# User-tian/Conan

Measured on AMD Instinct MI355X. Metric: chunks/sec (80 ms chunk, 16 kHz), all streams summed; p50 per-chunk latency beside it, higher is better.
Workload: dtype f32 (3×bf16-limb products, f32 accumulate)

## Files before the change

conan_amd/csrc/api.hip:

```cpp
#include "streams.h"

static thread_local std::string g_err;

template <typename F>
static int guarded(F&& f) {
  try {
    f();
    const hipError_t le = hipGetLastError();
    if (le != hipSuccess) throw ch::Error(CONAN_ERR_HIP, std::string("HIP launch error: ") + hipGetErrorString(le));
    return CONAN_OK;
  } catch (const ch::Error& e) {
    g_err = e.what();
    return e.code;
  } catch (const std::exception& e) {
    g_err = e.what();
    return CONAN_ERR_INVALID;
  }
}

static void validate_cfg(const conan_cfg& c) {
  if (c.abi_version != CONAN_HIP_ABI_VERSION) throw Error(CONAN_ERR_INVALID, "conan_cfg.abi_version mismatch");
  if (c.models & CONAN_MODEL_HIFIGAN) {
    if (c.voc_num_ups < 1 || c.voc_num_ups > CONAN_MAX_UPS) throw Error(CONAN_ERR_INVALID, "voc_num_ups");
    if (c.voc_num_resblocks < 1 || c.voc_num_resblocks > 3) throw Error(CONAN_ERR_UNSUPPORTED, "1..3 resblock branches supported");
// ... 187 lines not shown
}

int conan_streams_create_opts(conan_ctx* ctx, int max_slots, int max_frames, int max_ref_frames, const conan_streams_opts* opts,
                              conan_streams** out) {
  return guarded([&] {
    if (!ctx || !out) throw Error(CONAN_ERR_INVALID, "null argument");
    int arith = CONAN_ARITH_AUTO, flags = 0;
    if (opts) {
      if (opts->abi_version != CONAN_HIP_ABI_VERSION) throw Error(CONAN_ERR_INVALID, "conan_streams_opts.abi_version mismatch");
      for (int r : opts->reserved) if (r != 0) throw Error(CONAN_ERR_INVALID, "conan_streams_opts.reserved must be 0");
      arith = opts->arith; flags = opts->flags;
      if (opts->reserved0 != 0) throw Error(CONAN_ERR_INVALID, "conan_streams_opts.reserved0 must be 0");
      if (flags & ~(CONAN_STREAMS_FUSED_DECODER_BLOCKS | CONAN_STREAMS_SEPARATE_SMALL_STEPS | CONAN_STREAMS_FIXED_PLAN | CONAN_STREAMS_SHARED_DEVICE)) throw Error(CONAN_ERR_INVALID, "conan_streams_opts.flags: unknown bits");
      if (arith != CONAN_ARITH_AUTO && arith != CONAN_ARITH_F32 && arith != CONAN_ARITH_LIMB) throw Error(CONAN_ERR_INVALID, "conan_streams_opts.arith: 0 (auto), 1 (f32) or 2 (limb)");
    }
    if (!ctx->finalized) throw Error(CONAN_ERR_STATE, "conan_ctx_finalize must run before conan_streams_create");
    if (max_slots < 1 || max_frames < 1) throw Error(CONAN_ERR_INVALID, "max_slots / max_frames");
    HIP_CHECK(hipSetDevice(ctx->device));
    conan_streams* s = new conan_streams();
    try {
      s->parse_dev_plan(opts ? opts->dev_plan : nullptr);
      s->fixed_plan = (flags & CONAN_STREAMS_FIXED_PLAN) != 0; s->shared_device = (flags & CONAN_STREAMS_SHARED_DEVICE) != 0;
      s->ctx = ctx; s->live = &device_live_streams(ctx->device); s->live->fetch_add(1); s->max_slots = max_slots; s->max_frames = std::max(max_frames, ctx->cfg.emf_segment); s->max_ref = std::max(4, max_ref_frames);
      s->d_slots = (int*)s->alloc(max_slots + cnk::kSlotTablePad); s->d_ident = (int*)s->alloc(max_slots + 1); s->d_zero = (int*)s->alloc(max_slots);
      s->d_lens = (int*)s->alloc(max_slots); s->d_lens2 = (int*)s->alloc(max_slots);
      s->d_codes = (int*)s->alloc((size_t)max_slots * s->max_frames * 2);
      s->sk_slab_floats = 8ll << 20; s->sk_max_tiles = 4096;
      for (int w = 0; w < 3; ++w) { s->sk_slab[w] = s->alloc((size_t)s->sk_slab_floats); s->sk_counters[w] = (int*)s->alloc(s->sk_max_tiles); }
      for (int w = 0; w < 2; ++w) s->rb_sched[w] = (int*)s->alloc(4);
      for (int w = 0; w < 3; ++w) s->cp_ticket[w] = (int*)s->alloc(4);
      { const char* e = s->dev("RESERVE_CUS"); s->reserve_cus = e ? atoi(e) : 0; }
      { const char* e = s->dev("ROWCONV"); s->use_rowconv = !(e && e[0] == '0'); }
      s->rb_merge = s->dev("RB_NOMERGE") == nullptr;
      if (arith == CONAN_ARITH_LIMB && !((ctx->cfg.models & CONAN_MODEL_HIFIGAN) && ctx->has_limb_weights))
        throw Error(CONAN_ERR_UNSUPPORTED, "arith = limb: this context holds no bf16-limb weights (no HiFi-GAN model, or a vocoder configuration without limb kernels)");
      s->arith_auto = arith == CONAN_ARITH_AUTO;
      s->rb_limb = arith == CONAN_ARITH_LIMB || (arith == CONAN_ARITH_AUTO && ctx->has_limb_weights && s->dev("RB_NOLIMB") == nullptr);
      s->opt_flags = flags;
      s->mega_single = !(s->opt_flags & CONAN_STREAMS_SEPARATE_SMALL_STEPS);
      { const char* e = s->dev("FENCED"); s->fenced = e && e[0] == '1'; }
      { const char* e = s->dev("DEC_MEGA"); s->use_mega = !(e && e[0] == '0'); }
      { const char* e = s->dev("MEGA_GRID"); if (e && atoi(e) > 0) s->mega_grid = std::min(atoi(e), ctx->num_cu); }
      { const char* e = s->dev("FRONT_CUSTRIDE"); if (e && atoi(e) >= 2) s->use_mega = false; }
      { const char* e = s->dev("MEGA_GS"); if (e && (atoi(e) == 4 || atoi(e) == 8 || atoi(e) == 16)) s->mega_gs = atoi(e); }
      { const char* e = s->dev("MEGA_NARROW"); if (e && e[0] == '0') s->mega_narrow_ksplit = false; }
      s->mega_bar = reinterpret_cast<unsigned*>(s->alloc(16 * (size_t)(ctx->num_cu + 2)));
      s->mega_x = reinterpret_cast<unsigned*>(s->alloc(256 + 32 * 64));

      {
        HIP_CHECK(hipHostMalloc((void**)&s->h_guard, 64, hipHostMallocMapped));
        memset(s->h_guard, 0, 64);
        unsigned* hdev = nullptr;
        HIP_CHECK(hipHostGetDevicePointer((void**)&hdev, s->h_guard, 0));
        s->d_guard = reinterpret_cast<unsigned*>(s->alloc(16));
        HIP_CHECK(hipMemcpy(s->d_guard + 2, &hdev, sizeof(hdev), hipMemcpyHostToDevice));
      }
      s->slot_seen.assign(max_slots, 0); s->has_ref.assign(max_slots, 0); s->voice_of.assign(max_slots, -1); s->voc_fresh.assign(max_slots, 1); s->wav_out.voc_samples.assign(max_slots, 0); s->wav_in.in_fmt.assign(max_slots, 0); s->wav_out.out_fmt.assign(max_slots, 0);
      s->pin.init((size_t)max_slots + cnk::kSlotTablePad);
      s->pos_emf = (int*)s->alloc(max_slots); s->pos_dec = (int*)s->alloc(max_slots); s->pos_voc = (int*)s->alloc(max_slots);
      std::vector<int> id(max_slots);
      for (int i = 0; i < max_slots; ++i) id[i] = i;
      HIP_CHECK(hipMemcpy(s->d_ident, id.data(), max_slots * sizeof(int), hipMemcpyHostToDevice));
      s->wav_in.fe_slot.assign(max_slots, conan_streams::FeSlot());
      if ((ctx->cfg.models & 7) == 7) {
        const int seg = ctx->cfg.emf_segment, rc = ctx->cfg.emf_right_context, hop = ctx->hop;
        s->wav_in.fe_LA = ch::next_pow2(2048 + seg * hop);
// ... 578 lines not shown
```

conan_amd/csrc/kernels.h:

```cpp
#pragma once
#include <hip/hip_runtime.h>
#include <stdint.h>
#include <stdlib.h>

#include "voice_layout.h"

namespace cnk {

inline const char* dev_getenv(const char* name) {
#ifdef CONAN_DEV_SWITCHES
  return getenv(name);
#else
  (void)name;
  return nullptr;
#endif
}
#define HIP_CHECK(x) ::ch::hip_check((x), #x)


struct TRef {
  float* base;
  long long slot_stride;
  int C;
  int lmask;
// ... 102 lines not shown
  const int* assign;
  int assign_per;
  int wr_max;
  float* slab; int* counters;
  long long slab_floats; int max_counters;
};
bool conv_limb_supported(const ConvArgs& a);
int conv_limb_shape(const ConvArgs* p, int nprob, int num_cu, int plan_n = 0, bool tail_split = false);
bool launch_conv_limb(const ConvLimbGroup& g, int shape, int num_cu, hipStream_t st);
int conv_limb_tail_slices(const ConvArgs& a, int shape, int num_cu);
const char* conv_limb_name(int shape);

struct RBProb {
  const float* w1; const float* w2;
  const float* b1; const float* b2;
  const unsigned short* w1l; const unsigned short* w2l;
  TRef x;
  TRef y;
  int k, dil;
};
struct RBArgs {
  RBProb p[3];
  const int* slots; const int* pos;
  const int* tiles;
  int ntiles;
  int* sched;
  int nprob, n, T;
  int tiles_per_slot;
  int order[3];
  float slope;
  int merge;
  TRef ymean;
  unsigned long long* dbg;
};
bool resblock_fused_supported(int C, int kmax, int span_max);
int resblock_fused_rows(int C, int T, int n, int ksum, int kmax, int num_cu);
bool launch_resblock_fused(const RBArgs& a, int C, int rows, int num_cu, hipStream_t st);
bool resblock_fused_can_merge(int C, int rows);
const char* resblock_fused_name(int C, int rows, bool merge = false);
const int* resblock_tiles(const RBArgs& a, int ro, int* total_out);
bool resblock_limb_supported(int C, int kmax, int span_max);
constexpr int kResblockLimbMaxSlots = 256;
int resblock_limb_rows(int C, int span_max);
bool launch_resblock_limb(const RBArgs& a, int C, int rows, int num_cu, hipStream_t st);
bool resblock_limb_can_merge(int C, int rows);
const char* resblock_limb_name(int C, int rows, bool merge = false);


struct RPProb {
  const float* w1; const float* w2;
  const float* b1; const float* b2;
  TRef x, y;
  TRef xh;
  int k, dil;
};
struct RPArgs {
  RPProb p[3];
  const int* slots; const int* pos;
  const int* tiles; int ntiles;
  int* sched;
  float* xb;
  unsigned* xflag; unsigned* mbox; unsigned* xcount;
  int nprob, n, T;
  float slope;
  unsigned* guard;
  int fault;
// ... 414 lines not shown
```

conan_amd/csrc/resblock_limb.hip:

```cpp
#include <algorithm>
#include <cstring>
#include <type_traits>

#include "kernels.h"

#define RL_MAX_SLOTS 256

#ifndef RL_HELPER_PRIO
#define RL_HELPER_PRIO 3
#endif
#ifndef RL_MATRIX_PRIO
#define RL_MATRIX_PRIO 0
#endif
#ifndef RL_STAMPS
#define RL_STAMPS 0
#endif

#ifdef RL_ABLATE_W
#define RL_WOFF(x) 0
#define RL_WOFF2(a_, b_) (b_)
#else
#define RL_WOFF(x) (x)
#define RL_WOFF2(a_, b_) (a_)
#endif
// ... 177 lines not shown
            __builtin_amdgcn_sched_group_barrier(0x100, 1, 0);
          }
        } else {
          __builtin_amdgcn_sched_group_barrier(0x008, NRW * NCW, 0);
        }
      }
      __builtin_amdgcn_sched_group_barrier(0x020, 3 * NCW, 0);
      __builtin_amdgcn_sched_barrier(0);
    }
  }
}

}

#define RL_SEL(br_, f) ((br_) == 0 ? a.p[0].f : ((br_) == 1 ? a.p[1].f : a.p[2].f))

template <int C, int NR2, int SPAN, bool MERGE>
__global__ __launch_bounds__(512, 2) void resblock_limb_kernel(const RBArgs a) {
  using G = RLGeom<C, NR2, SPAN>;
  constexpr int LDB = G::LDB;
  __shared__ __attribute__((aligned(16))) u16 lds[G::LDS_U16 + 16 + 4 * RL_MAX_SLOTS];
  u16* const win = lds;
  u16* const xt = lds + 3 * G::PLW;
  float* const accimg = reinterpret_cast<float*>(xt);
  int* const meta = reinterpret_cast<int*>(lds + G::LDS_U16);
  int* const sptab = meta + 8;
  const int tid = threadIdx.x;
  const int lane = tid & 63;
  const int wave = __builtin_amdgcn_readfirstlane(tid >> 6);
  const int ntiles = a.ntiles;
  const float slope = a.slope;
  const int T = a.T;
  constexpr bool merge = MERGE;
  const int np = a.nprob;

  if (wave >= 4) {
    const int ht = tid - 256;
    __builtin_amdgcn_s_setprio(RL_HELPER_PRIO);
    auto hbar = [&]() __attribute__((always_inline)) { asm volatile("s_waitcnt lgkmcnt(0)\n\ts_barrier" ::: "memory"); };
    constexpr int NIT = (G::WR_MAX * G::C4 + 255) / 256;
    float4 wv[NIT];
    int wtotal = 0, wzr = 0;
    auto win_issue = [&](const int p, const int i, const int t0, const int slot, const int pos) __attribute__((always_inline)) {
      const int k = RL_SEL(p, k), d = RL_SEL(p, dil);
      const int wr = G::XT_ROWS + (k - 1) * d;
      const int tw0 = t0 - (k - 1) - (k - 1) * d;
      const int xmode = a.p[0].x.mode, xrate = a.p[0].x.rate;
      const float* xb = RL_SEL(p, x.base) + (long long)(xmode == 0 ? slot : i) * RL_SEL(p, x.slot_stride);
      const unsigned rbase = (xmode == 0 ? (unsigned)pos * (unsigned)xrate : 0u) + (unsigned)(RL_SEL(p, x.off) + tw0);
      const unsigned rmask = xmode == 0 ? (unsigned)RL_SEL(p, x.lmask) : 0xffffffffu;
      wtotal = wr * G::C4;
#pragma unroll
      for (int u = 0; u < NIT; ++u) {
        const int idx = ht + 256 * u;
        const int w = idx / G::C4, c4 = idx - w * G::C4;
        const unsigned row = (rbase + (unsigned)w) & rmask;
        wv[u] = idx < wtotal ? rl_gload4(xb + (long long)row * C + c4 * 4) : make_float4(0.f, 0.f, 0.f, 0.f);
      }
      const long long abs0 = (xmode == 0 ? (long long)pos * xrate : 0ll) + t0 - (k - 1);
      wzr = abs0 >= 0 ? 0 : (abs0 < -(long long)G::XT_ROWS ? G::XT_ROWS : (int)-abs0);
    };
    auto win_write = [&]() __attribute__((always_inline)) {
#pragma unroll
      for (int u = 0; u < NIT; ++u) {
        const int idx = ht + 256 * u;
        const int w = idx / G::C4, c4 = idx - w * G::C4;
        unsigned h[2], m[2], l[2];
        rl_split2(rl_lrelu2((f32x2){wv[u].x, wv[u].y}, slope), h[0], m[0], l[0]);
        rl_split2(rl_lrelu2((f32x2){wv[u].z, wv[u].w}, slope), h[1], m[1], l[1]);
        if (idx < wtotal) {
          u16* dst = win + w * LDB + c4 * 4;
          *reinterpret_cast<uint2*>(dst) = make_uint2(h[0], h[1]);
          *reinterpret_cast<uint2*>(dst + G::PLW) = make_uint2(m[0], m[1]);
          *reinterpret_cast<uint2*>(dst + 2 * G::PLW) = make_uint2(l[0], l[1]);
        }
      }
      if (ht == 0) meta[0] = wzr;
    };
    constexpr int NOUT = (G::RO * G::C4) / 256;
// ... 43 lines not shown
          else {
            float4 sm = osum[MERGE ? u : 0];
            if (op == 0) sm = v; else { sm.x += v.x; sm.y += v.y; sm.z += v.z; sm.w += v.w; }
            osum[MERGE ? u : 0] = sm;
            if (op == np - 1) {
              const float dn = (float)np;
              if (np > 1) { sm.x /= dn; sm.y /= dn; sm.z /= dn; sm.w /= dn; }
              sm.x = sm.x > 0.f ? sm.x : sm.x * slope; sm.y = sm.y > 0.f ? sm.y : sm.y * slope;
              sm.z = sm.z > 0.f ? sm.z : sm.z * slope; sm.w = sm.w > 0.f ? sm.w : sm.w * slope;
              rl_gstore4(oyb + (long long)((oyr0 + (unsigned)r) & oym) * oyC + oc4 * 4, sm);
            }
          }
        }
      }
    };
#if RL_STAMPS
    const unsigned long long h_t0 = __builtin_amdgcn_s_memtime();
    unsigned long long h_t[6] = {0, 0, 0, 0, 0, 0};
#define RL_HT(i_) h_t[i_] = __builtin_amdgcn_s_memtime() - h_t0
#else
#define RL_HT(i_)
#endif
    int dv0 = 0;
    if (wave == 4 && lane == 0) dv0 = __hip_atomic_fetch_add(a.sched, 1, __ATOMIC_RELAXED, __HIP_MEMORY_SCOPE_AGENT);
    for (int e = ht; e < a.n; e += 256) {
      const int sl = a.slots ? *(gci)(a.slots + e) : e;
      sptab[2 * e] = sl; sptab[2 * e + 1] = a.pos ? *(gci)(a.pos + sl) : 0;
    }
    const int tps = a.tiles_per_slot, per_prob = a.n * tps;
    auto decode = [&](const int e, int& p, int& i, int& t0) __attribute__((always_inline)) {
      if constexpr (!MERGE) {
        const int b = e / per_prob, rem = e - b * per_prob;
        p = b == 0 ? a.order[0] : (b == 1 ? a.order[1] : a.order[2]);
        i = rem / tps; t0 = (rem - i * tps) * G::RO;
      } else {
        const int g = e / np;
        p = e - g * np; i = g / tps; t0 = (g - i * tps) * G::RO;
      }
    };
    int cur = -1, p = -1, i = 0, t0 = 0;
    if (wave == 4) {
      cur = __builtin_amdgcn_readfirstlane(dv0) * (merge ? np : 1);
      if (cur >= ntiles) cur = -1;
      if (cur >= 0) decode(cur, p, i, t0);
      if (lane == 0) { meta[1] = cur; meta[2] = p; meta[3] = 0; }
    }
    RL_HT(0);
    asm volatile("s_waitcnt lgkmcnt(0)\n\ts_barrier" ::: "memory");
    RL_HT(1);
    if (wave != 4) {
      cur = __builtin_amdgcn_readfirstlane(meta[1]);
      if (cur >= 0) decode(cur, p, i, t0);
    }
    if (cur >= 0) {
    int slot = __builtin_amdgcn_readfirstlane(sptab[2 * i]), pos = __builtin_amdgcn_readfirstlane(sptab[2 * i + 1]);
    win_issue(p, i, t0, slot, pos);
    RL_HT(2);
    int gen = 1;
    int dv = 0, dnext = -1;
    auto draw_issue = [&](const int have, const int idx_prev, const int p_prev) __attribute__((always_inline)) {
      if (wave == 4 && lane == 0 && have) {
        if (merge && p_prev != np - 1) dnext = idx_prev + 1;
        else { dnext = -1; dv = __hip_atomic_fetch_add(a.sched, 1, __ATOMIC_RELAXED, __HIP_MEMORY_SCOPE_AGENT); }
      }
    };
    auto draw_take = [&](const int have) __attribute__((always_inline)) {
      int idx = -1;
      if (!have) return idx;
      if (wave == 4) {
        const int drawn = dv * (merge ? np : 1);
        idx = __builtin_amdgcn_readfirstlane(dnext >= 0 ? dnext : drawn);
        if (idx >= ntiles) idx = -1;
        if (lane == 0) {
          meta[1] = idx;
          asm volatile("s_waitcnt lgkmcnt(0)" ::: "memory");
          __hip_atomic_store(&meta[3], gen, __ATOMIC_RELEASE, __HIP_MEMORY_SCOPE_WORKGROUP);
        }
      } else {
        while (__hip_atomic_load(&meta[3], __ATOMIC_ACQUIRE, __HIP_MEMORY_SCOPE_WORKGROUP) != gen) __builtin_amdgcn_s_sleep(4);
        idx = __builtin_amdgcn_readfirstlane(meta[1]);
      }
      ++gen;
      return idx;
    };
    const bool deep = ntiles >= 5 * (int)gridDim.x * (merge ? np : 1);
    auto stage = [&](const int e) __attribute__((always_inline)) {
      int pe, ie, te;
      decode(e, pe, ie, te);
      win_issue(pe, ie, te, __builtin_amdgcn_readfirstlane(sptab[2 * ie]), __builtin_amdgcn_readfirstlane(sptab[2 * ie + 1]));
      return pe;
    };
    int nxt = -1, pn = -1;
    if (deep) {
      draw_issue(1, cur, p);
      nxt = draw_take(1);
    }
    RL_HT(3);
    win_write();
    RL_HT(4);
    hbar();
    RL_HT(5);
#if RL_STAMPS
    if (a.dbg && blockIdx.x == 0 && wave == 4 && lane == 0) { unsigned long long* q = a.dbg + 256 * 4 + 12; for (int e = 0; e < 6; ++e) q[e] = h_t[e]; }
#endif
    bool pending = false;
    for (;;) {
      const bool have = deep ? nxt >= 0 : true;
      if (deep && nxt >= 0) pn = stage(nxt);
      draw_issue(have, deep ? nxt : cur, deep ? pn : p);
      if (pending) out_store();
      int nn = -1;
      if (!deep) {
        nxt = draw_take(have); pn = -1;
        if (nxt >= 0) pn = stage(nxt);
      }
      if (ht == 0) meta[2] = nxt >= 0 ? pn : -1;
      hbar();
      hbar();
      if (nxt >= 0) win_write();
      hbar();
      hbar();
      out_fetch(p, i, t0, slot, pos);
      pending = true;
      if (deep) nn = draw_take(have);
      if (nxt < 0) break;
      cur = nxt;
      decode(cur, p, i, t0);
      slot = __builtin_amdgcn_readfirstlane(sptab[2 * i]); pos = __builtin_amdgcn_readfirstlane(sptab[2 * i + 1]);
      nxt = nn;
    }
    if (pending) out_store();
    }
    if (ht == 0) {
      const int d = __hip_atomic_fetch_add(a.sched + 1, 1, __ATOMIC_RELAXED, __HIP_MEMORY_SCOPE_AGENT);
      if (d == (int)gridDim.x - 1) {
        __hip_atomic_store(a.sched, 0, __ATOMIC_RELAXED, __HIP_MEMORY_SCOPE_AGENT);
        __hip_atomic_store(a.sched + 1, 0, __ATOMIC_RELAXED, __HIP_MEMORY_SCOPE_AGENT);
      }
    }
    return;
  }

  if (RL_MATRIX_PRIO) __builtin_amdgcn_s_setprio(RL_MATRIX_PRIO);
  auto bar = [&]() __attribute__((always_inline)) { asm volatile("s_waitcnt lgkmcnt(0)\n\ts_barrier" ::: "memory"); };
  const int wc = wave % (4 / G::RSPLIT);
  const int wr = wave / (4 / G::RSPLIT);
  const int ct0 = wc * G::NCW;
  const int lr = lane & 15, lg = lane >> 4;
#if RL_STAMPS
  unsigned long long st_gemm = 0, st_t0 = __builtin_amdgcn_s_memtime(), st_r0 = __builtin_amdgcn_s_memrealtime(), st_bar = 0, st_b3 = 0, st_b1 = 0, st_b4 = 0, st_b2 = 0, st_e1 = 0, st_e2 = 0, st_tiles = 0, st_head = 0, st_pre = 0, st_mid = 0;
#define RL_T() __builtin_amdgcn_s_memtime()
#define RL_BAR(acc_) do { const unsigned long long q0_ = RL_T(); bar(); const unsigned long long q1_ = RL_T(); acc_ += q1_ - q0_; st_bar += q1_ - q0_; } while (0)
#define RL_GEMM(...) do { const unsigned long long s0_ = RL_T(); __VA_ARGS__; asm volatile("s_nop 0" ::"v"(acc[0][0][0])); st_gemm += RL_T() - s0_; } while (0)
#else
#define RL_BAR(acc_) bar()
#define RL_GEMM(...) __VA_ARGS__
#endif
  f32x4 bw[G::RING][G::NCW][3];
  bar();
  int p = __builtin_amdgcn_readfirstlane(meta[2]);
  if (p < 0) return;
  {
    const long long cs = (long long)(RL_SEL(p, k) + 1) * G::KB * G::BLK;
    rl_prefetch_w<G::NCW, G::RING>(bw, RL_SEL(p, w1l) + (long long)ct0 * cs + lane * 8, cs);
  }
  bar();
#if RL_STAMPS
  st_head = RL_T() - st_t0;
#endif
  while (p >= 0) {
#if RL_STAMPS
    const unsigned long long top_ = RL_T();
#endif
    const int k = RL_SEL(p, k), d = RL_SEL(p, dil);
    const u16* const w1 = RL_SEL(p, w1l);
    const u16* const w2 = RL_SEL(p, w2l);
    const float* const b1 = RL_SEL(p, b1);
    const long long ct_stride = (long long)(k + 1) * G::KB * G::BLK;
    const int zrows = __builtin_amdgcn_readfirstlane(meta[0]);
    f32x4 b1v[G::NCW];
#pragma unroll
    for (int c = 0; c < G::NCW; ++c) b1v[c] = rl_gload(b1 + (ct0 + c) * 16 + 4 * lg);
    int pn;
    {
      f32x4 acc[G::NRW1][G::NCW];
#pragma unroll
      for (int r = 0; r < G::NRW1; ++r)
#pragma unroll
        for (int c = 0; c < G::NCW; ++c) acc[r][c] = (f32x4){0.f, 0.f, 0.f, 0.f};
      const int rt0 = wr * G::NRW1;
#if RL_STAMPS
      st_pre += RL_T() - top_;
#endif
      RL_GEMM(rl_gemm<G::NRW1, G::NCW, LDB, G::KB, G::RING>(win, G::PLW, rt0 * 16, d, k, w1 + (long long)ct0 * ct_stride + lane * 8, ct_stride,
                                                           w2 + (long long)ct0 * ct_stride + lane * 8, ct_stride, acc, bw, lane));
      RL_BAR(st_b3);
#if RL_STAMPS
      const unsigned long long e1_0 = RL_T();
#endif
      auto epilogue1 = [&](auto zr_c) __attribute__((always_inline)) {
        constexpr bool ZR = decltype(zr_c)::value;
#pragma unroll
        for (int c = 0; c < G::NCW; ++c) {
          const int col = (ct0 + c) * 16 + 4 * lg;
#pragma unroll
          for (int r = 0; r < G::NRW1; ++r) {
            if (rt0 + r < G::NR1) {
              const int m = (rt0 + r) * 16 + lr;
              unsigned h[2], mm[2], l[2];
              const f32x4 v = acc[r][c] + b1v[c];
              rl_split2(rl_lrelu2((f32x2){v[0], v[1]}, slope), h[0], mm[0], l[0]);
              rl_split2(rl_lrelu2((f32x2){v[2], v[3]}, slope), h[1], mm[1], l[1]);
              const bool zr = ZR && m < zrows;
              u16* dst = xt + m * LDB + col;
              *reinterpret_cast<uint2*>(dst) = zr ? make_uint2(0u, 0u) : make_uint2(h[0], h[1]);
              *reinterpret_cast<uint2*>(dst + G::PLX) = zr ? make_uint2(0u, 0u) : make_uint2(mm[0], mm[1]);
              *reinterpret_cast<uint2*>(dst + 2 * G::PLX) = zr ? make_uint2(0u, 0u) : make_uint2(l[0], l[1]);
            }
          }
        }
      };
      if (zrows > 0) epilogue1(std::true_type{}); else epilogue1(std::false_type{});
#if RL_STAMPS
      asm volatile("s_waitcnt lgkmcnt(0)" ::: "memory"); st_e1 += RL_T() - e1_0; ++st_tiles;
#endif
    }
    RL_BAR(st_b1);
#if RL_STAMPS
    const unsigned long long mid_ = RL_T();
#endif
    pn = __builtin_amdgcn_readfirstlane(meta[2]);
    const int pnx = pn >= 0 ? pn : p;
    const long long csn = (long long)(RL_SEL(pnx, k) + 1) * G::KB * G::BLK;
    const u16* const w1n = RL_SEL(pnx, w1l) + (long long)ct0 * csn + lane * 8;
    {
      f32x4 acc[G::NRW2][G::NCW];
#pragma unroll
      for (int r = 0; r < G::NRW2; ++r)
#pragma unroll
        for (int c = 0; c < G::NCW; ++c) acc[r][c] = (f32x4){0.f, 0.f, 0.f, 0.f};
      const int rt0 = wr * G::NRW2;
#if RL_STAMPS
      st_mid += RL_T() - mid_;
#endif
      RL_GEMM(rl_gemm<G::NRW2, G::NCW, LDB, G::KB, G::RING>(xt, G::PLX, rt0 * 16, 1, k, w2 + (long long)ct0 * ct_stride + lane * 8, ct_stride,
                                                           w1n, csn, acc, bw, lane));
      RL_BAR(st_b4);
#if RL_STAMPS
      const unsigned long long e2_0 = RL_T();
#endif
#pragma unroll
      for (int c = 0; c < G::NCW; ++c) {
        const int col = (ct0 + c) * 16 + 4 * lg;
#pragma unroll
        for (int r = 0; r < G::NRW2; ++r) {
          if (rt0 + r < NR2) *reinterpret_cast<f32x4*>(accimg + ((rt0 + r) * 16 + lr) * G::LDA + col) = acc[r][c];
        }
      }
#if RL_STAMPS
      asm volatile("s_waitcnt lgkmcnt(0)" ::: "memory"); st_e2 += RL_T() - e2_0;
#endif
    }
    RL_BAR(st_b2);
    p = pn;
  }
#if RL_STAMPS
  if (a.dbg && tid == 0) {
    unsigned long long* o = a.dbg + blockIdx.x * 4;
    if (blockIdx.x == 0) { unsigned long long* q = a.dbg + 256 * 4; q[0] = st_b3; q[1] = st_b1; q[2] = st_b4; q[3] = st_b2; q[4] = st_e1; q[5] = st_e2; q[6] = st_tiles; q[7] = st_gemm; q[8] = __builtin_amdgcn_s_memtime() - st_t0; q[9] = st_head; q[10] = st_pre; q[11] = st_mid; }
    o[0] = st_gemm; o[1] = __builtin_amdgcn_s_memtime() - st_t0; o[2] = __builtin_amdgcn_s_memrealtime() - st_r0; o[3] = st_bar;
  }
#endif
}


namespace {
struct RLCand { int C, NR2, span; };
const RLCand kLimbCands[] = {{32, 10, 50}, {64, 5, 50}, {128, 2, 50}};
}

bool resblock_limb_supported(int C, int kmax, int span_max) {
  for (const RLCand& c : kLimbCands)
    if (c.C == C && span_max <= c.span) return kmax <= 16;
  return false;
}

int resblock_limb_rows(int C, int span_max) {
  int best = 0;
  for (const RLCand& c : kLimbCands)
    if (c.C == C && span_max <= c.span) best = std::max(best, 16 * c.NR2);
  return best;
}

template <int C, int NR2, int SPAN, bool MERGE = false>
static bool launch_rl(const RBArgs& ain, int num_cu, hipStream_t st) {
  RBArgs a = ain;
  const int ro = 16 * NR2;
  a.tiles_per_slot = (a.T + ro - 1) / ro;
  const int total = a.nprob * a.n * a.tiles_per_slot;
  if (total <= 0) return true;
  if (!a.sched) return false;
  for (int p = 0; p < a.nprob; ++p) if (!a.p[p].w1l || !a.p[p].w2l) return false;
  if (a.n > RL_MAX_SLOTS) return false;
  if (!(a.slope > 0.f && a.slope <= 1.f)) return false;
  for (int p = 0; p < 3; ++p) a.order[p] = p;
  std::stable_sort(a.order, a.order + a.nprob, [&](int x, int y) { return a.p[x].k > a.p[y].k; });
  const int grid = std::min(a.merge ? total / a.nprob : total, num_cu);
  a.tiles = nullptr; a.ntiles = total;
  hipLaunchKernelGGL((resblock_limb_kernel<C, NR2, SPAN, MERGE>), dim3(grid), dim3(512), 0, st, a);
  return true;
}

bool launch_resblock_limb(const RBArgs& a, int C, int rows, int num_cu, hipStream_t st) {
  const int nr2 = rows / 16;
  if (a.merge) {
    if (C == 32 && nr2 == 10) return launch_rl<32, 10, 50, true>(a, num_cu, st);
    if (C == 64 && nr2 == 5) return launch_rl<64, 5, 50, true>(a, num_cu, st);
    if (C == 128 && nr2 == 2) return launch_rl<128, 2, 50, true>(a, num_cu, st);
    return false;
  }
  if (C == 32 && nr2 == 10) return launch_rl<32, 10, 50>(a, num_cu, st);
  if (C == 64 && nr2 == 5) return launch_rl<64, 5, 50>(a, num_cu, st);
  if (C == 128 && nr2 == 2) return launch_rl<128, 2, 50>(a, num_cu, st);
  return false;
}

bool resblock_limb_can_merge(int C, int rows) { return (C == 32 && rows == 160) || (C == 64 && rows == 80) || (C == 128 && rows == 32); }

const char* resblock_limb_name(int C, int rows, bool merge) {
  static thread_local char buf[72];
  const int span = 50;
  snprintf(buf, sizeof(buf), "cnk::resblock_limb_kernel<%d, %d, %d, %s>", C, rows / 16, span, merge ? "true" : "false");
  return buf;
}

}
```

conan_amd/csrc/streams.h:

```cpp
#pragma once
#include <array>
#include <functional>

#include "host_common.h"
#include "snapshot_layout.h"
#include "voice_layout.h"

using ch::Error;
using ch::Lin;
using ch::PackedConv;
using ch::Ring;
using cnk::ConvArgs;
using cnk::ConvGroup;
using cnk::TRef;

constexpr int kMaxBranches = 3;
constexpr int PADR = 16;

struct VocStage {
  Ring up;
  Ring upa;
  Ring xs;
  std::vector<std::vector<Ring>> xt, xo;
  std::vector<std::vector<Ring>> xa;
// ... 67 lines not shown
  const char* dev(const char* name) const {
    if (!dev_plan.empty()) {
      auto it = dev_plan.find(name);
      if (it != dev_plan.end()) return it->second.c_str();
    }
#ifdef CONAN_DEV_SWITCHES
    return getenv((std::string("CONAN_") + name).c_str());
#else
    return nullptr;
#endif
  }
  bool fixed_plan = false;
  bool in_style_pass = false;
  int plan_n(int n) const { return (fixed_plan && !in_style_pass) ? max_slots : n; }
  bool pipe_idle = false;
  bool shared_device = false;
  int max_slots = 0, max_frames = 0, max_ref = 0, S_max = 0;
  std::vector<void*> allocs;
  int64_t state_bytes = 0;
  std::vector<std::pair<float*, long long>> voc_state, dec_state, emf_state;

  int* d_slots = nullptr;
  int* d_ident = nullptr;
  int* d_zero = nullptr;
  int* d_lens = nullptr;
  int* d_lens2 = nullptr;
  int* d_codes = nullptr;
  float* sk_slab[3] = {nullptr, nullptr, nullptr};
  int* sk_counters[3] = {nullptr, nullptr, nullptr};
  int reserve_cus = 0;
  bool fenced = false;
  bool rb_limb = false;
  bool arith_auto = true;
  bool rb_merge = true;
  int* cp_ticket[3] = {nullptr, nullptr, nullptr};
  int* rb_sched[2] = {nullptr, nullptr};
  float* rp_xb[2] = {nullptr, nullptr};
  unsigned* rp_words[2] = {nullptr, nullptr};
  long long sk_slab_floats = 0;
  int sk_max_tiles = 0;
  std::vector<int> h_slots;
  std::vector<int> slot_seen;
  int slot_gen = 0;
  PinRing pin;
  int* pos_emf = nullptr; int* pos_dec = nullptr; int* pos_voc = nullptr;
  unsigned* d_guard = nullptr;
  unsigned* h_guard = nullptr;
  int test_fault = 0;
  void check_fault() const {
    if (!h_guard) return;
    const unsigned code = *(volatile const unsigned*)h_guard;
    if (code == 0) return;
    static const char* what[] = {"?", "decoder_mega_kernel group / grid barrier", "emformer_fused_kernel cluster exchange", "resblock_pair_kernel partner flag", "resblock_pair_kernel tile mailbox",
                                 "(retired)", "decoder_mega_kernel xcd election", "decoder_mega_kernel xcd roll call", "decoder_mega_kernel xcd flag barrier"};
    throw ch::Error(CONAN_ERR_HIP, std::string("a cross-workgroup wait gave up after its 50 ms budget (") + what[code < 9 ? code : 0] +
                                       "): results since then are invalid and this stream-set is unusable - destroy it and create a new one");
  }

  struct FeSlot { long long recv = 0; int frames = 0, chunks = 0, phase = 0; };
  struct RsSlot { const ch::RsTable* f = nullptr; long long in = 0, out = 0; int phase = 0; };
  struct WavIn {
    float* fe_audio = nullptr; float* fe_mel = nullptr; float* fe_chunk = nullptr;
    int fe_LA = 0, fe_LM = 0, fe_last_n = 0;
    std::vector<FeSlot> fe_slot;
    StageSets<RgRow> rg_sets;
    int* rg_codes[kStageSets] = {}; float* rg_mel[kStageSets] = {}; float* rg_wav[kStageSets] = {};
// ... 305 lines not shown
```

conan_amd/csrc/streams.hip:

```cpp
#include <climits>

#include "streams.h"


ConvArgs conan_streams::mk(const PackedConv& pc, const TRef& x, const TRef& y, int n, int T, const int* pos, int dil,
                           int pad_left) const {
  ConvArgs a;
  memset(&a, 0, sizeof(a));
  a.x = x;
  a.y = y; a.res = ch::null_ref(); a.m1 = ch::null_ref(); a.m2 = ch::null_ref();
  a.w = pc.w; a.bias = pc.bias; a.bvec = nullptr; a.slots = d_slots; a.pos = pos; a.lens = nullptr;
  a.Cin = pc.Cin; a.Cin_pad = pc.Cin_pad; a.Cin_alloc = pc.Cin_alloc; a.Cout = pc.Cout; a.Cout_pad = pc.Cout_pad;
  a.ktaps = pc.k; a.dil = dil; a.pad_left = pad_left < 0 ? (pc.k - 1) * dil : pad_left;
  a.T = T; a.n = n; a.in_act = cnk::ACT_NONE; a.in_slope = 0.f; a.out_act = cnk::ACT_NONE; a.out_scale = 1.f; a.out_slope = 0.f;
  a.shuffle_r = pc.shuffle_r;
  a.wl = reinterpret_cast<const unsigned short*>(pc.wl);
  if (x.C != pc.Cin && !(x.C > pc.Cin)) throw Error(CONAN_ERR_SHAPE, "conv input width mismatch");
  return a;
}

int conan_streams::pick_cfg(int M, int N, int nprob) const {
  const int wide[] = {cnk::CFG_64x64, cnk::CFG_32x64_K2, cnk::CFG_32x32_K4};
  const int narrow[] = {cnk::CFG_128x32, cnk::CFG_64x32_K2, cnk::CFG_32x32_K4};
  const int* order = N <= 32 ? narrow : wide;
// ... 127 lines not shown
      }
    }
    if (a.w2) {
      if ((v != 0 && v != 2) || (a.ktaps * (a.Cin >> 4)) % 8 != 0) { mega_rec_ok = false; return; }
      op.type = cnk::MOP_FFN;
      const int hc = a.Cout / mega_ffn_gs;
      op.u.rc.hid_overlay = hc == 64 ? 1 : 0;
      ldsf = op.u.rc.hid_overlay ? std::max(op.u.rc.wr_max * (a.Cin + 8), 16 * (hc + 8)) : op.u.rc.wr_max * (a.Cin + 8) + 16 * (hc + 8);
      mega_rec_flops += 2.0 * (double)a.n * a.T * a.Cout * a.Cout2;
    }
    mega_rec_flops += fl;
    mega_push(op, cnk::decoder_mega_lds_floats(op, ldsf));
    return;
  }
  const int prows = fixed_plan ? plan_n(a.n) * a.T : 0;
  profiled(cnk::rowconv_kernel_name(a, prows), fl, st, [&] { cnk::launch_rowconv(a, st, prows); });
}

bool conan_streams::launch_rb(const cnk::RBArgs& ain, int C, hipStream_t st, const TRef* ymean) {
  cnk::RBArgs a = ain;
  a.sched = rb_sched[ws_index(st) == 1 ? 1 : 0];
  int ksum = 0, kmax = 0;
  double fl = 0.0;
  for (int p = 0; p < a.nprob; ++p) { ksum += a.p[p].k; kmax = std::max(kmax, a.p[p].k); fl += 2.0 * 2.0 * (double)a.n * a.T * C * C * a.p[p].k; }
  const int cus = std::max(8, ctx->num_cu - (ws_index(st) == 1 ? reserve_cus : 0));
  int span = 0;
  bool limb = rb_limb;
  for (int p = 0; p < a.nprob; ++p) { span = std::max(span, (a.p[p].k - 1) * a.p[p].dil); limb = limb && a.p[p].w1l && a.p[p].w2l; }
  limb = limb && plan_n(a.n) <= cnk::kResblockLimbMaxSlots && cnk::resblock_limb_supported(C, kmax, span);
  const int rows = limb ? cnk::resblock_limb_rows(C, span) : cnk::resblock_fused_rows(C, a.T, plan_n(a.n), ksum, kmax, cus);
  const long long groups = (long long)plan_n(a.n) * ((a.T + rows - 1) / rows);
  const long long rounds = (groups + cus - 1) / cus;
  const bool balanced = groups * 10 >= rounds * cus * 9;
  a.merge = (ymean && rb_merge && a.nprob > 1 && groups >= cus && balanced && (limb ? cnk::resblock_limb_can_merge(C, rows) : cnk::resblock_fused_can_merge(C, rows))) ? 1 : 0;
  if (a.merge) a.ymean = *ymean;
  profiled(limb ? cnk::resblock_limb_name(C, rows, a.merge != 0) : cnk::resblock_fused_name(C, rows, a.merge != 0), fl, st, [&] {
    if (!(limb ? cnk::launch_resblock_limb(a, C, rows, cus, st) : cnk::launch_resblock_fused(a, C, rows, cus, st))) throw Error(CONAN_ERR_HIP, "fused resblock launch failed");
  });
  return a.merge != 0;
}

void conan_streams::launch_rp(const cnk::RPArgs& ain, hipStream_t st) {
  cnk::RPArgs a = ain;
  const int w = ws_index(st) == 1 ? 1 : 0;
  const int pairs = ctx->num_cu / 2;
  a.xb = rp_xb[w]; a.xflag = rp_words[w]; a.mbox = rp_words[w] + (size_t)pairs * 8; a.xcount = rp_words[w] + (size_t)pairs * 12;
  a.sched = reinterpret_cast<int*>(rp_words[w] + (size_t)pairs * 14);
  a.guard = d_guard; a.fault = test_fault == 3 ? 1 : 0;
  if (test_fault == 3) test_fault = 0;
  double fl = 0.0;
  for (int p = 0; p < a.nprob; ++p) fl += 2.0 * 2.0 * (double)a.n * a.T * 256.0 * 256.0 * a.p[p].k;
  profiled(cnk::resblock_pair_name(a.T), fl, st, [&] {
    if (!cnk::launch_resblock_pair(a, ctx->num_cu, st)) throw Error(CONAN_ERR_HIP, "resblock pair launch failed");
  });
}

void conan_streams::mega_print_stamps() {
  if (!mega_dbg || mega_dbg_prog < 0 || mega_dbg_prog >= (int)mega_cache.size()) return;
  (void)hipDeviceSynchronize();
  const MegaProgram& e = mega_cache[mega_dbg_prog];
  std::vector<unsigned long long> h(cnk::kMegaDbgWords);
  if (hipMemcpy(h.data(), mega_dbg, h.size() * 8, hipMemcpyDeviceToHost) != hipSuccess) return;
  static const char* names[] = {"rowconv<1,1,1>", "rowconv<1,1,4>", "rowlin", "layernorm", "xattn", "pitch_head", "embed", "copy32", "advance", "ffn"};
  constexpr int nnames = (int)(sizeof(names) / sizeof(names[0]));
  fprintf(stderr, "[decoder_mega] last launch: %d groups x %d workgroups, %d jobs, %d operators, %d group barriers, %.1f us in all (workgroup 0; first job per operator below)\n",
          e.groups, e.group_size, e.njobs, e.nops, e.barriers, (h[e.nops + 1] - h[0]) / 100.0);
// ... 19 lines not shown
  if (stamps && !mega_dbg) mega_dbg = reinterpret_cast<unsigned long long*>(alloc(2 * (size_t)cnk::kMegaDbgWords));
  if (stamps) HIP_CHECK(hipMemsetAsync(mega_dbg, 0, sizeof(unsigned long long) * cnk::kMegaDbgWords, st));
  if (stamps) mega_dbg_prog = (int)(&e - mega_cache.data());
  cnk::MegaLaunch m; memset(&m, 0, sizeof(m));
  m.prog = e.dev; m.nops = e.nops; m.njobs = e.njobs; m.groups = e.groups; m.group_size = e.group_size; m.kw4 = e.kw4; m.lds_bytes = e.lds_bytes;
  m.slots = d_slots; m.pos = pos_dec; m.n = e.n; m.T = e.T;
  m.gbar = mega_bar + 16; m.bar = mega_bar; m.bar_base = mega_bar_count; m.dbg = mega_dbg; m.guard = d_guard; m.wide_regs = rb_limb ? 1 : 0;
  m.xcd = e.xcd ? 1 : 0;
  const bool pipelined = st_front != nullptr && st == st_front;
  if (e.xcd) {
    static const bool pad_always = ch::dev_getenv("CONAN_MEGA_XCD_PAD") != nullptr;
    if (pipelined && !pad_always) m.lds_bytes = e.lds_need;
    mega_xseq = mega_xseq + 1u;
    m.xs = mega_x; m.xseq = mega_xseq; m.xdec_base = mega_xdec;
    if (test_fault == 1) { m.xseq += 7u; mega_xseq += 7u; test_fault = 0; }
    profiled("cnk::decoder_mega_kernel<4, 2>", e.flops, st, [&] { cnk::launch_decoder_mega(m, st); });
    mega_xdec += (unsigned)(e.groups * e.group_size);
    return;
  }
  if (test_fault == 1) { m.bar_base += 1u; test_fault = 0; }
  mega_gseq = mega_gseq + 1u;
  m.xs = mega_x; m.xseq = mega_gseq;
  { const bool nol2 = dev("MEGA_NOL2") != nullptr;
    const char* lay = dev("MEGA_LAYOUT");
    const bool mfast = lay && lay[0] == 'm';
    m.xdec_base = (nol2 ? 1u : 0u) | (mfast ? 2u : 0u); }
  profiled(rb_limb ? "cnk::decoder_mega_kernel<4, 3>" : "cnk::decoder_mega_kernel<6, 3>", e.flops, st, [&] { cnk::launch_decoder_mega(m, st); });
  mega_bar_count += (unsigned)(e.groups * e.group_size);
}

void conan_streams::parse_dev_plan(const char* text) {
  static const char* known[] = {"RESERVE_CUS", "ROWCONV", "RB_NOMERGE", "RB_NOLIMB", "FENCED", "DEC_MEGA", "MEGA_GRID", "FRONT_CUSTRIDE", "EMF_CUSTRIDE", "MEGA_GS",
                                "MEGA_NARROW", "MEGA_NOL2", "MEGA_LAYOUT", "FRONT_PRIO", "RB_UNFUSED", "RB_FUSED", "RB_PAIR", "RB_NOPAIR", "RP_MIN_SLOTS",
                                "UPS_CFG", "EMF_CLUSTER", "EMF_UNFUSED", "NO_TALL", "TALL_MAXT"};
  dev_plan.clear();
  if (!text) return;
  const std::string t(text);
  size_t p = 0;
  while (p < t.size()) {
    size_t q = t.find(';', p);
    if (q == std::string::npos) q = t.size();
    std::string item = t.substr(p, q - p);
    p = q + 1;
    while (!item.empty() && item.front() == ' ') item.erase(item.begin());
    while (!item.empty() && item.back() == ' ') item.pop_back();
    if (item.empty()) continue;
    const size_t eq = item.find('=');
    const std::string name = item.substr(0, eq), value = eq == std::string::npos ? "1" : item.substr(eq + 1);
    bool ok = false;
    for (const char* k : known) ok = ok || name == k;
    if (!ok) throw Error(CONAN_ERR_INVALID, "conan_streams_opts.dev_plan: unknown switch '" + name + "'");
    dev_plan[name] = value;
  }
}

void conan_streams::set_slots(const int32_t* slots, int n, hipStream_t st) {
  if (n <= 0 || n > max_slots) throw Error(CONAN_ERR_INVALID, "slot count out of range");
  bool same = (int)h_slots.size() == n;
  for (int i = 0; i < n; ++i) {
    if (slots[i] < 0 || slots[i] >= max_slots) throw Error(CONAN_ERR_INVALID, "slot index out of range");
    if (same && h_slots[i] != slots[i]) same = false;
  }
  if (same) return;
  if (++slot_gen == 0x7fffffff) { std::fill(slot_seen.begin(), slot_seen.end(), 0); slot_gen = 1; }
  for (int i = 0; i < n; ++i) {
    if (slot_seen[slots[i]] == slot_gen) throw Error(CONAN_ERR_INVALID, "duplicate slot");
    slot_seen[slots[i]] = slot_gen;
  }
  h_slots.assign(slots, slots + n);
  std::vector<int> up(h_slots); up.resize((size_t)n + cnk::kSlotTablePad, h_slots.back());
  pin.upload(d_slots, up.data(), up.size(), st);
}


void conan_streams::async_init() {
  if (st_front) return;
  {
    int lo = 0, hi = 0;
    HIP_CHECK(hipDeviceGetStreamPriorityRange(&lo, &hi));
    const char* e = dev("FRONT_PRIO");
    const int mode = e ? atoi(e) : 0;
    auto masked = [&](hipStream_t* st, const char* env) {
      const char* v = dev(env);
      const int stride = v ? atoi(v) : 0;
// ... 444 lines not shown
```

Baseline: 47160.

## Chain consecutive time tiles into runs in the limb resblock kernel, carrying conv halos

For the non-merged C=128 limb resblock kernel, adjacent time tiles of the same slot are grouped into runs of length up to two and processed by the same workgroup. The first conv's activation halo rows are parked in LDS and reused by the next tile, so that tile loads a shorter input window and skips recomputing the halo rows. Run length is chosen on the host from the average work per CU and can be overridden through a dev switch. The cost is fewer schedulable work items, which can hurt load balance, plus added control logic and LDS traffic for parking.

```diff
diff --git a/conan_amd/csrc/api.hip b/conan_amd/csrc/api.hip
--- a/conan_amd/csrc/api.hip
+++ b/conan_amd/csrc/api.hip
@@ -243,6 +243,7 @@
       { const char* e = s->dev("RESERVE_CUS"); s->reserve_cus = e ? atoi(e) : 0; }
       { const char* e = s->dev("ROWCONV"); s->use_rowconv = !(e && e[0] == '0'); }
       s->rb_merge = s->dev("RB_NOMERGE") == nullptr;
+      if (const char* rr = s->dev("RL_RUN")) s->rl_run = strcmp(rr, "auto") == 0 ? 0 : (atoi(rr) > 0 ? atoi(rr) : -1);
       if (arith == CONAN_ARITH_LIMB && !((ctx->cfg.models & CONAN_MODEL_HIFIGAN) && ctx->has_limb_weights))
         throw Error(CONAN_ERR_UNSUPPORTED, "arith = limb: this context holds no bf16-limb weights (no HiFi-GAN model, or a vocoder configuration without limb kernels)");
       s->arith_auto = arith == CONAN_ARITH_AUTO;
diff --git a/conan_amd/csrc/kernels.h b/conan_amd/csrc/kernels.h
--- a/conan_amd/csrc/kernels.h
+++ b/conan_amd/csrc/kernels.h
@@ -158,6 +158,11 @@
   int merge;
   TRef ymean;
   unsigned long long* dbg;
+  int run_req, plan_n;
+  int run_len[3];
+  int run_cnt[3];
+  int run_end[3];
+  int nitems;
 };
 bool resblock_fused_supported(int C, int kmax, int span_max);
 int resblock_fused_rows(int C, int T, int n, int ksum, int kmax, int num_cu);
diff --git a/conan_amd/csrc/resblock_limb.hip b/conan_amd/csrc/resblock_limb.hip
--- a/conan_amd/csrc/resblock_limb.hip
+++ b/conan_amd/csrc/resblock_limb.hip
@@ -233,6 +233,9 @@
   const float slope = a.slope;
   const int T = a.T;
   constexpr bool merge = MERGE;
+  constexpr bool RUNS = !MERGE && C == 128;
+  static_assert(!RUNS || G::RSPLIT == 1, "a carried tile's c1 is c2's register shape: every matrix wave holds all rows");
+  u16* const parkp = win + (G::WR_MAX - 16) * LDB;
   const int np = a.nprob;
 
   if (wave >= 4) {
@@ -242,10 +245,10 @@
     constexpr int NIT = (G::WR_MAX * G::C4 + 255) / 256;
     float4 wv[NIT];
     int wtotal = 0, wzr = 0;
-    auto win_issue = [&](const int p, const int i, const int t0, const int slot, const int pos) __attribute__((always_inline)) {
+    auto win_issue = [&](const int p, const int i, const int t0, const int slot, const int pos, const bool carried) __attribute__((always_inline)) {
       const int k = RL_SEL(p, k), d = RL_SEL(p, dil);
-      const int wr = G::XT_ROWS + (k - 1) * d;
-      const int tw0 = t0 - (k - 1) - (k - 1) * d;
+      const int wr = (RUNS && carried ? G::RO : G::XT_ROWS) + (k - 1) * d;
+      const int tw0 = t0 - (RUNS && carried ? 0 : k - 1) - (k - 1) * d;
       const int xmode = a.p[0].x.mode, xrate = a.p[0].x.rate;
       const float* xb = RL_SEL(p, x.base) + (long long)(xmode == 0 ? slot : i) * RL_SEL(p, x.slot_stride);
       const unsigned rbase = (xmode == 0 ? (unsigned)pos * (unsigned)xrate : 0u) + (unsigned)(RL_SEL(p, x.off) + tw0);
@@ -355,18 +358,39 @@
       if constexpr (!MERGE) {
         const int b = e / per_prob, rem = e - b * per_prob;
         p = b == 0 ? a.order[0] : (b == 1 ? a.order[1] : a.order[2]);
-        i = rem / tps; t0 = (rem - i * tps) * G::RO;
+        i = rem / tps;
+        const int tl = rem - i * tps;
+        t0 = tl * G::RO;
+        if constexpr (RUNS) {
+          const int L = b == 0 ? a.run_len[0] : (b == 1 ? a.run_len[1] : a.run_len[2]);
+          const int q = tl % L;
+          p |= (q != 0 ? 4 : 0) | ((q + 1 != L && tl + 1 != tps) ? 8 : 0);
+        }
       } else {
         const int g = e / np;
         p = e - g * np; i = g / tps; t0 = (g - i * tps) * G::RO;
       }
     };
+    auto item_tile = [&](const int it) __attribute__((always_inline)) {
+      if constexpr (!RUNS) return it;
+      else {
+        if (it >= a.nitems) return -1;
+        const int b = it >= a.run_end[0] ? (it >= a.run_end[1] ? 2 : 1) : 0;
+        const int rem = it - (b == 0 ? 0 : (b == 1 ? a.run_end[0] : a.run_end[1]));
+        const int R = b == 0 ? a.run_cnt[0] : (b == 1 ? a.run_cnt[1] : a.run_cnt[2]);
+        const int L = b == 0 ? a.run_len[0] : (b == 1 ? a.run_len[1] : a.run_len[2]);
+        const int i = rem / R;
+        return b * per_prob + i * tps + (rem - i * R) * L;
+      }
+    };
+#define RL_P(x_) (RUNS ? ((x_) & 3) : (x_))
     int cur = -1, p = -1, i = 0, t0 = 0;
     if (wave == 4) {
       cur = __builtin_amdgcn_readfirstlane(dv0) * (merge ? np : 1);
+      if (RUNS) cur = item_tile(cur);
       if (cur >= ntiles) cur = -1;
       if (cur >= 0) decode(cur, p, i, t0);
-      if (lane == 0) { meta[1] = cur; meta[2] = p; meta[3] = 0; }
+      if (lane == 0) { meta[1] = cur; meta[2] = cur >= 0 ? RL_P(p) : -1; meta[3] = 0; }
     }
     RL_HT(0);
     asm volatile("s_waitcnt lgkmcnt(0)\n\ts_barrier" ::: "memory");
@@ -377,13 +401,15 @@
     }
     if (cur >= 0) {
     int slot = __builtin_amdgcn_readfirstlane(sptab[2 * i]), pos = __builtin_amdgcn_readfirstlane(sptab[2 * i + 1]);
-    win_issue(p, i, t0, slot, pos);
+    win_issue(RL_P(p), i, t0, slot, pos, false);
     RL_HT(2);
     int gen = 1;
     int dv = 0, dnext = -1;
     auto draw_issue = [&](const int have, const int idx_prev, const int p_prev) __attribute__((always_inline)) {
       if (wave == 4 && lane == 0 && have) {
         if (merge && p_prev != np - 1) dnext = idx_prev + 1;
+        else if (RUNS && (p_prev & 8)) dv = -2 - idx_prev;
+        else if (RUNS) dv = __hip_atomic_fetch_add(a.sched, 1, __ATOMIC_RELAXED, __HIP_MEMORY_SCOPE_AGENT);
         else { dnext = -1; dv = __hip_atomic_fetch_add(a.sched, 1, __ATOMIC_RELAXED, __HIP_MEMORY_SCOPE_AGENT); }
       }
     };
@@ -391,8 +417,13 @@
       int idx = -1;
       if (!have) return idx;
       if (wave == 4) {
-        const int drawn = dv * (merge ? np : 1);
-        idx = __builtin_amdgcn_readfirstlane(dnext >= 0 ? dnext : drawn);
+        if constexpr (RUNS) {
+          const int v = __builtin_amdgcn_readfirstlane(dv);
+          idx = v < 0 ? -1 - v : item_tile(v);
+        } else {
+          const int drawn = dv * (merge ? np : 1);
+          idx = __builtin_amdgcn_readfirstlane(dnext >= 0 ? dnext : drawn);
+        }
         if (idx >= ntiles) idx = -1;
         if (lane == 0) {
           meta[1] = idx;
@@ -410,7 +441,7 @@
     auto stage = [&](const int e) __attribute__((always_inline)) {
       int pe, ie, te;
       decode(e, pe, ie, te);
-      win_issue(pe, ie, te, __builtin_amdgcn_readfirstlane(sptab[2 * ie]), __builtin_amdgcn_readfirstlane(sptab[2 * ie + 1]));
+      win_issue(RL_P(pe), ie, te, __builtin_amdgcn_readfirstlane(sptab[2 * ie]), __builtin_amdgcn_readfirstlane(sptab[2 * ie + 1]), RUNS && (pe & 4));
       return pe;
     };
     int nxt = -1, pn = -1;
@@ -437,13 +468,13 @@
         nxt = draw_take(have); pn = -1;
         if (nxt >= 0) pn = stage(nxt);
       }
-      if (ht == 0) meta[2] = nxt >= 0 ? pn : -1;
+      if (ht == 0) meta[2] = nxt >= 0 ? (RUNS ? pn & 7 : pn) : -1;
       hbar();
       hbar();
       if (nxt >= 0) win_write();
       hbar();
       hbar();
-      out_fetch(p, i, t0, slot, pos);
+      out_fetch(RL_P(p), i, t0, slot, pos);
       pending = true;
       if (deep) nn = draw_take(have);
       if (nxt < 0) break;
@@ -483,6 +514,7 @@
   bar();
   int p = __builtin_amdgcn_readfirstlane(meta[2]);
   if (p < 0) return;
+  int carried = 0;
   {
     const long long cs = (long long)(RL_SEL(p, k) + 1) * G::KB * G::BLK;
     rl_prefetch_w<G::NCW, G::RING>(bw, RL_SEL(p, w1l) + (long long)ct0 * cs + lane * 8, cs);
@@ -504,7 +536,63 @@
     f32x4 b1v[G::NCW];
 #pragma unroll
     for (int c = 0; c < G::NCW; ++c) b1v[c] = rl_gload(b1 + (ct0 + c) * 16 + 4 * lg);
-    int pn;
+    int pn = -1;
+    int park = 0;
+    if (RUNS && carried) {
+      f32x4 acc[G::NRW2][G::NCW];
+#pragma unroll
+      for (int r = 0; r < G::NRW2; ++r)
+#pragma unroll
+        for (int c = 0; c < G::NCW; ++c) acc[r][c] = (f32x4){0.f, 0.f, 0.f, 0.f};
+#if RL_STAMPS
+      st_pre += RL_T() - top_;
+#endif
+      RL_GEMM(rl_gemm<G::NRW2, G::NCW, LDB, G::KB, G::RING>(win, G::PLW, 0, d, k, w1 + (long long)ct0 * ct_stride + lane * 8, ct_stride,
+                                                           w2 + (long long)ct0 * ct_stride + lane * 8, ct_stride, acc, bw, lane));
+      RL_BAR(st_b3);
+#if RL_STAMPS
+      const unsigned long long e1_0 = RL_T();
+#endif
+      pn = __builtin_amdgcn_readfirstlane(meta[2]);
+      park = pn >= 0 ? (pn >> 2) & 1 : 0;
+      int lr = lane & 15, lg = lane >> 4;
+      asm volatile("" : "+v"(lr), "+v"(lg));
+      if (lr < k - 1) {
+#pragma unroll
+        for (int c = 0; c < G::NCW; ++c)
+#pragma unroll
+          for (int pl = 0; pl < 3; ++pl) {
+            const int o = lr * LDB + (ct0 + c) * 16 + 4 * lg;
+            *reinterpret_cast<uint2*>(xt + pl * G::PLX + o) = *reinterpret_cast<const uint2*>(parkp + pl * G::PLW + o);
+          }
+      }
+      const int pr = (k - 1) + lr - 16;
+#pragma unroll
+      for (int c = 0; c < G::NCW; ++c) {
+        const int col = (ct0 + c) * 16 + 4 * lg;
+#pragma unroll
+        for (int r = 0; r < G::NRW2; ++r) {
+          const int m = (k - 1) + r * 16 + lr;
+          unsigned h[2], mm[2], l[2];
+          const f32x4 v = acc[r][c] + b1v[c];
+          rl_split2(rl_lrelu2((f32x2){v[0], v[1]}, slope), h[0], mm[0], l[0]);
+          rl_split2(rl_lrelu2((f32x2){v[2], v[3]}, slope), h[1], mm[1], l[1]);
+          u16* dst = xt + m * LDB + col;
+          *reinterpret_cast<uint2*>(dst) = make_uint2(h[0], h[1]);
+          *reinterpret_cast<uint2*>(dst + G::PLX) = make_uint2(mm[0], mm[1]);
+          *reinterpret_cast<uint2*>(dst + 2 * G::PLX) = make_uint2(l[0], l[1]);
+          if (r == G::NRW2 - 1 && park && pr >= 0) {
+            u16* pd = parkp + pr * LDB + col;
+            *reinterpret_cast<uint2*>(pd) = make_uint2(h[0], h[1]);
+            *reinterpret_cast<uint2*>(pd + G::PLW) = make_uint2(mm[0], mm[1]);
+            *reinterpret_cast<uint2*>(pd + 2 * G::PLW) = make_uint2(l[0], l[1]);
+          }
+        }
+      }
+#if RL_STAMPS
+      asm volatile("s_waitcnt lgkmcnt(0)" ::: "memory"); st_e1 += RL_T() - e1_0; ++st_tiles;
+#endif
+    } else
     {
       f32x4 acc[G::NRW1][G::NCW];
 #pragma unroll
@@ -521,6 +609,10 @@
 #if RL_STAMPS
       const unsigned long long e1_0 = RL_T();
 #endif
+      if constexpr (RUNS) {
+        pn = __builtin_amdgcn_readfirstlane(meta[2]);
+        park = pn >= 0 ? (pn >> 2) & 1 : 0;
+      }
       auto epilogue1 = [&](auto zr_c) __attribute__((always_inline)) {
         constexpr bool ZR = decltype(zr_c)::value;
 #pragma unroll
@@ -539,6 +631,12 @@
               *reinterpret_cast<uint2*>(dst) = zr ? make_uint2(0u, 0u) : make_uint2(h[0], h[1]);
               *reinterpret_cast<uint2*>(dst + G::PLX) = zr ? make_uint2(0u, 0u) : make_uint2(mm[0], mm[1]);
               *reinterpret_cast<uint2*>(dst + 2 * G::PLX) = zr ? make_uint2(0u, 0u) : make_uint2(l[0], l[1]);
+              if (RUNS && r == G::NRW1 - 1 && park && lr < k - 1) {
+                u16* pd = parkp + lr * LDB + col;
+                *reinterpret_cast<uint2*>(pd) = make_uint2(h[0], h[1]);
+                *reinterpret_cast<uint2*>(pd + G::PLW) = make_uint2(mm[0], mm[1]);
+                *reinterpret_cast<uint2*>(pd + 2 * G::PLW) = make_uint2(l[0], l[1]);
+              }
             }
           }
         }
@@ -552,7 +650,12 @@
 #if RL_STAMPS
     const unsigned long long mid_ = RL_T();
 #endif
-    pn = __builtin_amdgcn_readfirstlane(meta[2]);
+    if constexpr (!RUNS) pn = __builtin_amdgcn_readfirstlane(meta[2]);
+    else {
+      pn = __builtin_amdgcn_readfirstlane(pn);
+      carried = __builtin_amdgcn_readfirstlane(park);
+      if (pn >= 0) pn &= 3;
+    }
     const int pnx = pn >= 0 ? pn : p;
     const long long csn = (long long)(RL_SEL(pnx, k) + 1) * G::KB * G::BLK;
     const u16* const w1n = RL_SEL(pnx, w1l) + (long long)ct0 * csn + lane * 8;
@@ -614,6 +717,9 @@
     if (c.C == C && span_max <= c.span) best = std::max(best, 16 * c.NR2);
   return best;
 }
+
+static double run_frac(int C) { return C == 128 ? 0.9 : 0.0; }
+constexpr int kRunMax = 2;
 
 template <int C, int NR2, int SPAN, bool MERGE = false>
 static bool launch_rl(const RBArgs& ain, int num_cu, hipStream_t st) {
@@ -628,7 +734,23 @@
   if (!(a.slope > 0.f && a.slope <= 1.f)) return false;
   for (int p = 0; p < 3; ++p) a.order[p] = p;
   std::stable_sort(a.order, a.order + a.nprob, [&](int x, int y) { return a.p[x].k > a.p[y].k; });
-  const int grid = std::min(a.merge ? total / a.nprob : total, num_cu);
+  for (int b = 0; b < 3; ++b) { a.run_len[b] = 1; a.run_cnt[b] = a.tiles_per_slot; }
+  if (!MERGE && run_frac(C) > 0.0 && a.run_req >= 0) {
+    const int pn = a.plan_n > 0 ? a.plan_n : a.n;
+    int ksum = 0;
+    for (int p = 0; p < a.nprob; ++p) ksum += a.p[p].k;
+    const long long ptiles = (long long)a.nprob * pn * a.tiles_per_slot;
+    const double avg = (double)pn * a.tiles_per_slot * ksum / (double)std::max<long long>(1, std::min<long long>(ptiles, num_cu));
+    for (int b = 0; b < a.nprob; ++b) {
+      int L = a.run_req > 0 ? a.run_req : std::min(kRunMax, (int)(run_frac(C) * avg / a.p[a.order[b]].k));
+      L = std::max(1, std::min(L, a.tiles_per_slot));
+      a.run_cnt[b] = (a.tiles_per_slot + L - 1) / L;
+      a.run_len[b] = (a.tiles_per_slot + a.run_cnt[b] - 1) / a.run_cnt[b];
+    }
+  }
+  a.nitems = 0;
+  for (int b = 0; b < 3; ++b) { if (b < a.nprob) a.nitems += a.n * a.run_cnt[b]; a.run_end[b] = a.nitems; }
+  const int grid = std::min(a.merge ? total / a.nprob : a.nitems, num_cu);
   a.tiles = nullptr; a.ntiles = total;
   hipLaunchKernelGGL((resblock_limb_kernel<C, NR2, SPAN, MERGE>), dim3(grid), dim3(512), 0, st, a);
   return true;
diff --git a/conan_amd/csrc/streams.h b/conan_amd/csrc/streams.h
--- a/conan_amd/csrc/streams.h
+++ b/conan_amd/csrc/streams.h
@@ -123,6 +123,7 @@
   bool fenced = false;
   bool rb_limb = false;
   bool arith_auto = true;
+  int rl_run = 0;
   bool rb_merge = true;
   int* cp_ticket[3] = {nullptr, nullptr, nullptr};
   int* rb_sched[2] = {nullptr, nullptr};
diff --git a/conan_amd/csrc/streams.hip b/conan_amd/csrc/streams.hip
--- a/conan_amd/csrc/streams.hip
+++ b/conan_amd/csrc/streams.hip
@@ -183,6 +183,7 @@
   const long long groups = (long long)plan_n(a.n) * ((a.T + rows - 1) / rows);
   const long long rounds = (groups + cus - 1) / cus;
   const bool balanced = groups * 10 >= rounds * cus * 9;
+  a.run_req = rl_run; a.plan_n = plan_n(a.n);
   a.merge = (ymean && rb_merge && a.nprob > 1 && groups >= cus && balanced && (limb ? cnk::resblock_limb_can_merge(C, rows) : cnk::resblock_fused_can_merge(C, rows))) ? 1 : 0;
   if (a.merge) a.ymean = *ymean;
   profiled(limb ? cnk::resblock_limb_name(C, rows, a.merge != 0) : cnk::resblock_fused_name(C, rows, a.merge != 0), fl, st, [&] {
@@ -268,7 +269,7 @@
 void conan_streams::parse_dev_plan(const char* text) {
   static const char* known[] = {"RESERVE_CUS", "ROWCONV", "RB_NOMERGE", "RB_NOLIMB", "FENCED", "DEC_MEGA", "MEGA_GRID", "FRONT_CUSTRIDE", "EMF_CUSTRIDE", "MEGA_GS",
                                 "MEGA_NARROW", "MEGA_NOL2", "MEGA_LAYOUT", "FRONT_PRIO", "RB_UNFUSED", "RB_FUSED", "RB_PAIR", "RB_NOPAIR", "RP_MIN_SLOTS",
-                                "UPS_CFG", "EMF_CLUSTER", "EMF_UNFUSED", "NO_TALL", "TALL_MAXT"};
+                                "UPS_CFG", "EMF_CLUSTER", "EMF_UNFUSED", "NO_TALL", "TALL_MAXT", "RL_RUN"};
   dev_plan.clear();
   if (!text) return;
   const std::string t(text);
@@ -286,6 +287,11 @@
     bool ok = false;
     for (const char* k : known) ok = ok || name == k;
     if (!ok) throw Error(CONAN_ERR_INVALID, "conan_streams_opts.dev_plan: unknown switch '" + name + "'");
+    if (name == "RL_RUN") {
+      bool num = !value.empty() && value.size() <= 4;
+      for (char ch2 : value) num = num && ch2 >= '0' && ch2 <= '9';
+      if (!num && value != "auto") throw Error(CONAN_ERR_INVALID, "conan_streams_opts.dev_plan: RL_RUN is 0, auto or a run length, not '" + value + "'");
+    }
     dev_plan[name] = value;
   }
 }
```

After: 47210 (median of 3 runs). About the same (+0.1%).
